# codelion/adaptive-classifier

Measured on NVIDIA H100. Metric: queries/sec predict() bert-base 128-tok, 1M x 768 prototypes, higher is better.
Workload: dtype f16

## Files before the change

### adaptive_classifier_b200/csrc/common.cuh

```cuda
#pragma once

#include <cuda_runtime.h>
#include <cuda.h>
#include <stdint.h>
#include <stdio.h>
#include <string.h>
#include <string>

#include "../../include/adaptive_b200.h"

namespace ac {

void set_error(const char *fmt, ...);
int check_cuda(cudaError_t e, const char *what);

#define AC_CUDA(call)                                                \
    do {                                                             \
        int _rc = ::ac::check_cuda((call), #call);                   \
        if (_rc != 0) return _rc;                                    \
    } while (0)

#define AC_REQUIRE(cond, ...)                                        \
    do {                                                             \
        if (!(cond)) {                                               \
// ... 131 lines not shown
}
__device__ __forceinline__ void wgmma_m64n128_tf32(float (&d)[64], uint64_t a_desc, uint64_t b_desc, uint32_t accumulate) {
    asm volatile(
        "{\n\t"
        ".reg .pred p;\n\t"
        "setp.ne.b32 p, %66, 0;\n\t"
        "wgmma.mma_async.sync.aligned.m64n128k8.f32.tf32.tf32 "
        "{%0, %1, %2, %3, %4, %5, %6, %7, %8, %9, %10, %11, %12, %13, %14, %15, "
        "%16, %17, %18, %19, %20, %21, %22, %23, %24, %25, %26, %27, %28, %29, %30, %31, "
        "%32, %33, %34, %35, %36, %37, %38, %39, %40, %41, %42, %43, %44, %45, %46, %47, "
        "%48, %49, %50, %51, %52, %53, %54, %55, %56, %57, %58, %59, %60, %61, %62, %63}, "
        "%64, %65, p, 1, 1;\n\t"
        "}"
        : "+f"(d[0]), "+f"(d[1]), "+f"(d[2]), "+f"(d[3]), "+f"(d[4]), "+f"(d[5]), "+f"(d[6]), "+f"(d[7]),
          "+f"(d[8]), "+f"(d[9]), "+f"(d[10]), "+f"(d[11]), "+f"(d[12]), "+f"(d[13]), "+f"(d[14]), "+f"(d[15]),
          "+f"(d[16]), "+f"(d[17]), "+f"(d[18]), "+f"(d[19]), "+f"(d[20]), "+f"(d[21]), "+f"(d[22]), "+f"(d[23]),
          "+f"(d[24]), "+f"(d[25]), "+f"(d[26]), "+f"(d[27]), "+f"(d[28]), "+f"(d[29]), "+f"(d[30]), "+f"(d[31]),
          "+f"(d[32]), "+f"(d[33]), "+f"(d[34]), "+f"(d[35]), "+f"(d[36]), "+f"(d[37]), "+f"(d[38]), "+f"(d[39]),
          "+f"(d[40]), "+f"(d[41]), "+f"(d[42]), "+f"(d[43]), "+f"(d[44]), "+f"(d[45]), "+f"(d[46]), "+f"(d[47]),
          "+f"(d[48]), "+f"(d[49]), "+f"(d[50]), "+f"(d[51]), "+f"(d[52]), "+f"(d[53]), "+f"(d[54]), "+f"(d[55]),
          "+f"(d[56]), "+f"(d[57]), "+f"(d[58]), "+f"(d[59]), "+f"(d[60]), "+f"(d[61]), "+f"(d[62]), "+f"(d[63])
        : "l"(a_desc), "l"(b_desc), "r"(accumulate));
}
__device__ __forceinline__ void wgmma_m64n64_f16(float (&d)[32], uint64_t a_desc, uint64_t b_desc, uint32_t accumulate) {
    asm volatile(
        "{\n\t"
        ".reg .pred p;\n\t"
        "setp.ne.b32 p, %34, 0;\n\t"
        "wgmma.mma_async.sync.aligned.m64n64k16.f32.f16.f16 "
        "{%0, %1, %2, %3, %4, %5, %6, %7, %8, %9, %10, %11, %12, %13, %14, %15, "
        "%16, %17, %18, %19, %20, %21, %22, %23, %24, %25, %26, %27, %28, %29, %30, %31}, "
        "%32, %33, p, 1, 1, 0, 0;\n\t"
        "}"
        : "+f"(d[0]), "+f"(d[1]), "+f"(d[2]), "+f"(d[3]), "+f"(d[4]), "+f"(d[5]), "+f"(d[6]), "+f"(d[7]),
          "+f"(d[8]), "+f"(d[9]), "+f"(d[10]), "+f"(d[11]), "+f"(d[12]), "+f"(d[13]), "+f"(d[14]), "+f"(d[15]),
          "+f"(d[16]), "+f"(d[17]), "+f"(d[18]), "+f"(d[19]), "+f"(d[20]), "+f"(d[21]), "+f"(d[22]), "+f"(d[23]),
          "+f"(d[24]), "+f"(d[25]), "+f"(d[26]), "+f"(d[27]), "+f"(d[28]), "+f"(d[29]), "+f"(d[30]), "+f"(d[31])
        : "l"(a_desc), "l"(b_desc), "r"(accumulate));
}
__device__ __forceinline__ void wgmma_m64n32_f16(float (&d)[16], uint64_t a_desc, uint64_t b_desc, uint32_t accumulate) {
    asm volatile(
        "{\n\t"
        ".reg .pred p;\n\t"
        "setp.ne.b32 p, %18, 0;\n\t"
        "wgmma.mma_async.sync.aligned.m64n32k16.f32.f16.f16 "
        "{%0, %1, %2, %3, %4, %5, %6, %7, %8, %9, %10, %11, %12, %13, %14, %15}, "
        "%16, %17, p, 1, 1, 0, 0;\n\t"
        "}"
        : "+f"(d[0]), "+f"(d[1]), "+f"(d[2]), "+f"(d[3]), "+f"(d[4]), "+f"(d[5]), "+f"(d[6]), "+f"(d[7]),
          "+f"(d[8]), "+f"(d[9]), "+f"(d[10]), "+f"(d[11]), "+f"(d[12]), "+f"(d[13]), "+f"(d[14]), "+f"(d[15])
        : "l"(a_desc), "l"(b_desc), "r"(accumulate));
}

template <int NREG>
__device__ __forceinline__ void wgmma_store_acc(const float (&d)[NREG], float *tile, int ld) {
    const int t = threadIdx.x & 127;
    const int r0 = 16 * (t >> 5) + ((t & 31) >> 2), c0 = 2 * (t & 3);
#pragma unroll
    for (int j = 0; j < NREG / 4; ++j) {
        *reinterpret_cast<float2 *>(tile + r0 * ld + 8 * j + c0) = make_float2(d[4 * j], d[4 * j + 1]);
        *reinterpret_cast<float2 *>(tile + (r0 + 8) * ld + 8 * j + c0) = make_float2(d[4 * j + 2], d[4 * j + 3]);
    }
}
__device__ __forceinline__ void acc_row_ld32(const float *p, float (&v)[32]) {
#pragma unroll
    for (int j = 0; j < 32; j += 4) {
        const float4 x = *reinterpret_cast<const float4 *>(p + j);
        v[j] = x.x; v[j + 1] = x.y; v[j + 2] = x.z; v[j + 3] = x.w;
    }
}

int make_tmap_2d(CUtensorMap *out, const void *gptr, int elem_bytes, uint64_t rows, uint64_t cols,
                 uint64_t row_stride_bytes, uint32_t box_rows, uint32_t box_cols);

}
```

### adaptive_classifier_b200/csrc/encoder.cu

```cuda
#include "gemm_tc.cuh"
#include <cuda_fp16.h>
#include <math_constants.h>
#include <algorithm>
#include <array>
#include <type_traits>
#include <vector>

namespace ac {

__device__ __forceinline__ float ex2_approx(float x) {
    float y;
    asm("ex2.approx.ftz.f32 %0, %1;" : "=f"(y) : "f"(x));
    return y;
}
__device__ __forceinline__ float rcp_approx(float x) {
    float y;
    asm("rcp.approx.ftz.f32 %0, %1;" : "=f"(y) : "f"(x));
    return y;
}
__device__ __forceinline__ float gelu_erf(float y) {
    const float ay = fabsf(y);
    const float t = rcp_approx(fmaf(0.3275911f * 0.70710678118654752440f, ay, 1.f));
    float p = fmaf(0.5f * 1.061405429f, t, 0.5f * -1.453152027f);
    p = fmaf(p, t, 0.5f * 1.421413741f);
// ... 475 lines not shown
        if (i < nv) {
            const int col = (lane + 32 * i) * 4;
            const float4 a = __ldg(reinterpret_cast<const float4 *>(word + static_cast<int64_t>(id) * H + col));
            if (!pos) {
                x[i] = a;
                continue;
            }
            const float4 t = __ldg(reinterpret_cast<const float4 *>(type + static_cast<int64_t>(tt) * H + col));
            const float4 q = __ldg(reinterpret_cast<const float4 *>(pos + static_cast<int64_t>(p) * H + col));
            x[i].x = (a.x + t.x) + q.x;
            x[i].y = (a.y + t.y) + q.y;
            x[i].z = (a.z + t.z) + q.z;
            x[i].w = (a.w + t.w) + q.w;
        }
    ln_row(x, nv, H, w, b, eps, lane, F32_OUT ? out_full + static_cast<int64_t>(row) * H : nullptr,
           out_half + static_cast<int64_t>(row) * H);
}

__global__ void cls_normalize_kernel(const float *__restrict__ x, int B, int S, int H, float *__restrict__ out) {
    const int bq = blockIdx.x * (blockDim.x >> 5) + (threadIdx.x >> 5);
    const int lane = threadIdx.x & 31;
    if (bq >= B) return;
    const float *src = x + static_cast<int64_t>(bq) * S * H;
    float s = 0.f;
    for (int i = lane; i < H; i += 32) s = fmaf(src[i], src[i], s);
    const float nrm = fmaxf(sqrtf(warp_sum(s)), 1e-12f);
    for (int i = lane; i < H; i += 32) out[static_cast<int64_t>(bq) * H + i] = src[i] / nrm;
}

__global__ void gather_cls_kernel(const __half *__restrict__ ctx, const float *__restrict__ x, int B, int S, int H,
                                  __half *__restrict__ ctx_cls, float *__restrict__ x_cls) {
    const int bq = blockIdx.x * (blockDim.x >> 5) + (threadIdx.x >> 5);
    const int lane = threadIdx.x & 31;
    if (bq >= B) return;
    const int64_t src = static_cast<int64_t>(bq) * S * H, dst = static_cast<int64_t>(bq) * H;
    for (int i = lane; i < H / 8; i += 32)
        reinterpret_cast<uint4 *>(ctx_cls + dst)[i] = reinterpret_cast<const uint4 *>(ctx + src)[i];
    for (int i = lane; i < H / 4; i += 32)
        reinterpret_cast<float4 *>(x_cls + dst)[i] = reinterpret_cast<const float4 *>(x + src)[i];
}

__global__ void round_copy_kernel(const float *__restrict__ in, float *__restrict__ out, int64_t n, int do_round) {
    const int64_t stride = static_cast<int64_t>(gridDim.x) * blockDim.x;
    for (int64_t i = static_cast<int64_t>(blockIdx.x) * blockDim.x + threadIdx.x; i < n; i += stride)
        out[i] = do_round ? round_tf32(in[i]) : in[i];
}
__global__ void to_half_kernel(const float *__restrict__ in, __half *__restrict__ out, int64_t n) {
    const int64_t stride = static_cast<int64_t>(gridDim.x) * blockDim.x;
    for (int64_t i = static_cast<int64_t>(blockIdx.x) * blockDim.x + threadIdx.x; i < n; i += stride)
        out[i] = __float2half_rn(in[i]);
}

constexpr int ATT_THREADS = 128;
constexpr int ATT_S_LD = 128 + 4;
constexpr int ATT_S_BYTES = 128 * ATT_S_LD * 4;
constexpr int ATT_REGION_BYTES = (ATT_S_BYTES + 1023) / 1024 * 1024;
constexpr int ATT_OFF_VT = ATT_REGION_BYTES, ATT_OFF_BAR = ATT_OFF_VT + 16 * 1024, ATT_OFF_TERM = ATT_OFF_BAR + 64;
template <class Score>
constexpr int ATT_SMEM = ATT_OFF_TERM + Score::SMEM_BLOCK + 1024 ;

template <int DH>
__device__ __forceinline__ void att_scores(const uint8_t *sQ, const uint8_t *sK, float *sS) {
    const uint64_t bd = wgmma_desc_sw128(smem_u32(sK));
#pragma unroll 1
    for (int half = 0; half < 2; ++half) {
        float s[64];
        const uint64_t a = wgmma_desc_sw128(smem_u32(sQ + half * 8192));
        wgmma_fence();
#pragma unroll
        for (int k = 0; k < DH / 16; ++k) wgmma_m64n128_f16(s, a + 2 * k, bd + 2 * k, k != 0);
        wgmma_commit();
        wgmma_wait<0>();
        wgmma_store_acc(s, sS + half * 64 * ATT_S_LD, ATT_S_LD);
    }
}
template <int DH>
__device__ __forceinline__ void att_pv(const uint8_t *sP, const uint8_t *sVt, float (&o)[2][DH / 2], bool accumulate) {
#pragma unroll
    for (int half = 0; half < 2; ++half) {
        wgmma_fence();
#pragma unroll
        for (int slab = 0; slab < 2; ++slab) {
            const uint64_t a = wgmma_desc_sw128(smem_u32(sP + slab * 16384 + half * 8192));
            const uint64_t bd = wgmma_desc_sw128(smem_u32(sVt + slab * 8192));
#pragma unroll
            for (int k = 0; k < 4; ++k) {
                if constexpr (DH == 64) wgmma_m64n64_f16(o[half], a + 2 * k, bd + 2 * k, accumulate || (slab | k) != 0);
                else wgmma_m64n32_f16(o[half], a + 2 * k, bd + 2 * k, accumulate || (slab | k) != 0);
            }
        }
    }
    wgmma_commit();
    wgmma_wait<0>();
}
__device__ __forceinline__ void att_store_p(uint32_t sp_base, int qrow, int c, const uint32_t *pk) {
    const uint32_t prow = sp_base + (c >> 6) * 16384 + (qrow >> 3) * 1024 + (qrow & 7) * 128;
    const int ch0 = (c & 63) >> 3;
#pragma unroll
    for (int ch = 0; ch < 4; ++ch) {
        asm volatile("st.shared.v4.b32 [%0], {%1, %2, %3, %4};" ::"r"(prow + (((ch0 + ch) ^ (qrow & 7)) << 4)),
                     "r"(pk[4 * ch]), "r"(pk[4 * ch + 1]), "r"(pk[4 * ch + 2]), "r"(pk[4 * ch + 3])
                     : "memory");
    }
}
template <int DH>
__device__ __forceinline__ void att_write_row(const float *orow, float inv, __half *dst) {
#pragma unroll
    for (int c = 0; c < DH; c += 8) {
        const float4 a = *reinterpret_cast<const float4 *>(orow + c);
        const float4 b = *reinterpret_cast<const float4 *>(orow + c + 4);
// ... 3 lines not shown
        pk.x = *reinterpret_cast<uint32_t *>(&h0); pk.y = *reinterpret_cast<uint32_t *>(&h1);
        pk.z = *reinterpret_cast<uint32_t *>(&h2); pk.w = *reinterpret_cast<uint32_t *>(&h3);
        *reinterpret_cast<uint4 *>(dst + c) = pk;
    }
}

__device__ __forceinline__ uint32_t band_bits(int q, int k0, int w) {
    if (w <= 0) return 0xffffffffu;
    const int lo = q - w - k0, hi = q + w - k0;
    if (hi < 0 || lo > 31) return 0u;
    const uint32_t up = hi >= 31 ? 0xffffffffu : (2u << hi) - 1u;
    const uint32_t dn = lo <= 0 ? 0xffffffffu : ~((1u << lo) - 1u);
    return up & dn;
}

__device__ __forceinline__ void att_key_bits(const int32_t *mask, int64_t row0, int S, int key0, int q, int window, int lane,
                                             uint32_t (&kmask)[4]) {
#pragma unroll
    for (int w4 = 0; w4 < 4; ++w4) {
        const int key = key0 + 32 * w4 + lane;
        const bool ok = (key < S) && (!mask || mask[row0 + key] != 0);
        kmask[w4] = __ballot_sync(0xffffffffu, ok) & band_bits(q, key0 + 32 * w4, window);
    }
}
__device__ __forceinline__ void att_exp_pack(const float (&r)[32], uint32_t km, float scale_log2, float mxs, float &sum,
                                             uint32_t *pk) {
#pragma unroll
    for (int j = 0; j < 32; j += 2) {
        const float e0 = ((km >> j) & 1u) ? ex2_approx(fmaf(r[j], scale_log2, -mxs)) : 0.f;
        const float e1 = ((km >> (j + 1)) & 1u) ? ex2_approx(fmaf(r[j + 1], scale_log2, -mxs)) : 0.f;
        sum += e0 + e1;
        __half2 hh = __floats2half2_rn(e0, e1);
        pk[j >> 1] = *reinterpret_cast<uint32_t *>(&hh);
    }
}

struct AttCta {
    uint8_t *smem;
    uint8_t *term;
    int tid, h, heads;
    int q0, nblk;
};

struct ScorePlain {
    static constexpr int MIN_DH = 32;
    static constexpr bool ONE_BLOCK = true;
    static constexpr int SCALE_TERMS = 1;
    static constexpr bool EX2_ROWS = false;
    static constexpr int SMEM_BLOCK = 0, SMEM_STREAM = 0;
    __device__ __forceinline__ void init_barriers(const AttCta &) const {}
    __device__ __forceinline__ void begin(const AttCta &) const {}
    __device__ __forceinline__ void add_block_terms(const AttCta &, int) const {}
    __device__ __forceinline__ void row(float (&)[32], const AttCta &, int, float) const {}
    __device__ __forceinline__ void after_pv(const AttCta &, int) const {}
};

struct ScoreRelBias : ScorePlain {
    const float *rel_bias;
    static constexpr int MIN_DH = 64;
    static constexpr bool EX2_ROWS = true;
    static constexpr int ATT_BIAS_OFS = AC_ENCODER_MAX_S - 128;
    static constexpr int SMEM_BLOCK = 1024, SMEM_STREAM = (AC_ENCODER_MAX_S + 128) * 4;
    __device__ __forceinline__ void begin(const AttCta &cta) const {
        const float *row = rel_bias + cta.h * (2 * AC_ENCODER_MAX_S - 1);
        float *sB = reinterpret_cast<float *>(cta.term);
        for (int t = cta.tid; t < 128 * cta.nblk + 127; t += ATT_THREADS)
            sB[t] = __ldg(row + ATT_BIAS_OFS - cta.q0 + t) * 1.44269504088896340736f;
    }
    __device__ __forceinline__ void row(float (&r)[32], const AttCta &cta, int key, float scale_log2) const {
        const float *bq = reinterpret_cast<const float *>(cta.term) + 127 - cta.tid;
#pragma unroll
        for (int j = 0; j < 32; ++j) r[j] = fmaf(r[j], scale_log2, bq[key + j]);
    }
};

template <int DH, class Score>
__global__ void __launch_bounds__(ATT_THREADS)
attention_kernel(const __grid_constant__ CUtensorMap tmap_qk, const __grid_constant__ CUtensorMap tmap_vt,
                 const int32_t *__restrict__ mask, int B, int S, int heads, int H, int window, __half *__restrict__ ctx,
                 const __grid_constant__ Score score) {
    static_assert(Score::ONE_BLOCK && DH >= Score::MIN_DH, "score term not written for this kernel or head dimension");
    static_assert(2 * (ATT_SMEM<Score> + 1024) <= 228 * 1024, "two attention CTAs must fit one SM");
    extern __shared__ uint8_t smem_raw[];
    uint8_t *smem = reinterpret_cast<uint8_t *>((reinterpret_cast<uintptr_t>(smem_raw) + 1023) & ~uintptr_t(1023));
    uint8_t *sQ = smem;
    uint8_t *sK = smem + 16 * 1024;
    float *sS = reinterpret_cast<float *>(smem);
    uint8_t *sP = smem;
    uint8_t *sVt = smem + ATT_OFF_VT;
    uint64_t *bar_load = reinterpret_cast<uint64_t *>(smem + ATT_OFF_BAR);

    const int tid = threadIdx.x, warp = tid >> 5, lane = tid & 31;
    const int b = blockIdx.x / heads, h = blockIdx.x % heads;
    const int64_t row0 = static_cast<int64_t>(b) * S;
    const AttCta cta = {smem, smem + ATT_OFF_TERM, tid, h, heads, 0, 1};

    if (tid == 0) {
        tma_prefetch_desc(&tmap_qk);
        tma_prefetch_desc(&tmap_vt);
        mbar_init(bar_load, 1);
        fence_mbar_init();
    }
    __syncthreads();
    if (tid == 0) {
        mbar_arrive_expect_tx(bar_load, 48 * 1024);
        const int r = static_cast<int>(row0);
        tma_load_2d(sQ, &tmap_qk, bar_load, h * DH, r);
        tma_load_2d(sK, &tmap_qk, bar_load, H + h * DH, r);
        const int vrow = (b * heads + h) * DH;
        tma_load_2d(sVt, &tmap_vt, bar_load, 0, vrow);
        tma_load_2d(sVt + 8 * 1024, &tmap_vt, bar_load, 64, vrow);
    }
    score.begin(cta);
    mbar_wait_guarded(bar_load, 0);
    {
        float s0[64], s1[64];
        const uint64_t bd = wgmma_desc_sw128(smem_u32(sK));
        const uint64_t a0 = wgmma_desc_sw128(smem_u32(sQ)), a1 = wgmma_desc_sw128(smem_u32(sQ + 8192));
        wgmma_fence();
#pragma unroll
        for (int k = 0; k < DH / 16; ++k) wgmma_m64n128_f16(s0, a0 + 2 * k, bd + 2 * k, k != 0);
#pragma unroll
        for (int k = 0; k < DH / 16; ++k) wgmma_m64n128_f16(s1, a1 + 2 * k, bd + 2 * k, k != 0);
        wgmma_commit();
        wgmma_wait<0>();
        __syncthreads();
        wgmma_store_acc(s0, sS, ATT_S_LD);
        wgmma_store_acc(s1, sS + 64 * ATT_S_LD, ATT_S_LD);
    }
    __syncthreads();

    const int qrow = warp * 32 + lane;
    const float *srow = sS + qrow * ATT_S_LD;
    uint32_t kmask[4];
    att_key_bits(mask, row0, S, 0, qrow, window, lane, kmask);
    const float scale_log2 = rsqrtf(static_cast<float>(Score::SCALE_TERMS * DH)) * 1.44269504088896340736f;
    const float sl2 = Score::EX2_ROWS ? 1.f : scale_log2;
    float mx = -CUDART_INF_F;
#pragma unroll 1
    for (int c = 0; c < 128; c += 32) {
        float r[32];
        acc_row_ld32(srow + c, r);
        score.row(r, cta, c, scale_log2);
        const uint32_t km = c == 0 ? kmask[0] : c == 32 ? kmask[1] : c == 64 ? kmask[2] : kmask[3];
#pragma unroll
        for (int j = 0; j < 32; ++j)
            if ((km >> j) & 1u) mx = fmaxf(mx, r[j]);
    }
    float sum = 0.f;
    uint32_t pk[64];
#pragma unroll
    for (int ci = 0; ci < 4; ++ci) {
        float r[32];
        acc_row_ld32(srow + 32 * ci, r);
        score.row(r, cta, 32 * ci, scale_log2);
        att_exp_pack(r, kmask[ci], sl2, mx * sl2, sum, pk + 16 * ci);
    }
    __syncthreads();
    const uint32_t sp_base = smem_u32(sP);
#pragma unroll
    for (int ci = 0; ci < 4; ++ci) att_store_p(sp_base, qrow, 32 * ci, pk + 16 * ci);
    fence_proxy_async_smem();
    __syncthreads();

    float o[2][DH / 2];
    att_pv<DH>(sP, sVt, o, false);
    __syncthreads();
    wgmma_store_acc(o[0], sS, ATT_S_LD);
    wgmma_store_acc(o[1], sS + 64 * ATT_S_LD, ATT_S_LD);
    __syncthreads();
    const float inv = (sum > 0.f) ? 1.f / sum : 0.f;
    if (qrow < S) att_write_row<DH>(srow, inv, ctx + (row0 + qrow) * H + h * DH);
}

constexpr int ATTS_STAGE_BYTES = 16 * 1024;
constexpr int ATTS_OFF_K = 16 * 1024, ATTS_OFF_VT = 48 * 1024, ATTS_OFF_P = 80 * 1024, ATTS_OFF_S = 112 * 1024;
constexpr int ATTS_OFF_BAR = ATTS_OFF_S + ATT_S_BYTES + 128 * 4, ATTS_OFF_TERM = ATTS_OFF_BAR + 2 * 8;
template <class Score>
constexpr int ATTS_SMEM = ATTS_OFF_TERM + Score::SMEM_STREAM + 1024 ;

constexpr int ATTS_POS_DELTAS = 2 * (AC_ENCODER_MAX_S / 128) - 1;

template <bool P2C>
__device__ __forceinline__ void att_rel_term(const uint8_t *sA, const uint8_t *sG, float *sS) {
    const int t = threadIdx.x & 127;
    const int r0 = 16 * (t >> 5) + ((t & 31) >> 2), c0 = 2 * (t & 3);
#pragma unroll 1
    for (int half = 0; half < 2; ++half) {
#pragma unroll 1
        for (int nc = 0; nc < 2; ++nc) {
            float c[64];
            const uint64_t a = wgmma_desc_sw128(smem_u32(sA + half * 8192));
            const uint64_t bd = wgmma_desc_sw128(smem_u32(sG + nc * 16384));
            wgmma_fence();
#pragma unroll
            for (int k = 0; k < 4; ++k) wgmma_m64n128_f16(c, a + 2 * k, bd + 2 * k, k != 0);
            wgmma_commit();
            wgmma_wait<0>();
#pragma unroll
            for (int j = 0; j < 64; ++j) {
                const int row = 64 * half + r0 + 8 * ((j >> 1) & 1);
                const int other = row - (128 * nc + 8 * (j >> 2) + c0 + (j & 1)) + 127;
                if (other >= 0 && other < 128) {
                    float *dst = P2C ? sS + other * ATT_S_LD + row : sS + row * ATT_S_LD + other;
                    *dst += c[j];
                }
            }
        }
    }
}

struct ScoreDisent : ScorePlain {
    CUtensorMap tmap_pos;
    int pos_row0;
    static constexpr int MIN_DH = 64;
    static constexpr bool ONE_BLOCK = false;
    static constexpr int SCALE_TERMS = 3;
    static constexpr int OFF_G = (ATTS_OFF_TERM + 2 * 8 + 1023) / 1024 * 1024 - ATTS_OFF_TERM;
    static constexpr int SMEM_STREAM = OFF_G + 2 * ATTS_STAGE_BYTES;
    __device__ __forceinline__ void issue_pos(const AttCta &cta, int i, int term) const {
        const int row =
            pos_row0 + (((static_cast<int>(blockIdx.y) - i + ATTS_POS_DELTAS / 2) * cta.heads + cta.h) * 2 + term) * 256;
        uint64_t *bar = reinterpret_cast<uint64_t *>(cta.term) + term;
        uint8_t *dst = term ? cta.smem + ATTS_OFF_P : cta.term + OFF_G;
        mbar_arrive_expect_tx(bar, 2 * ATTS_STAGE_BYTES);
// ... 174 lines not shown
}

__global__ void pos_gather_kernel(const float *__restrict__ pos_key, const float *__restrict__ pos_query,
                                  const int32_t *__restrict__ rel_index, int span, int heads, int H, __half *__restrict__ out) {
    const int64_t row = static_cast<int64_t>(blockIdx.x) * 4 + (threadIdx.x >> 6);
    const int col = threadIdx.x & 63;
    const int t = static_cast<int>(row % 256), term = static_cast<int>((row / 256) % 2);
    const int h = static_cast<int>((row / 512) % heads);
    const int64_t ld = row / (512 * static_cast<int64_t>(heads));
    const int d = static_cast<int>(ld % ATTS_POS_DELTAS);
    const int64_t l = ld / ATTS_POS_DELTAS;
    float v = 0.f;
    if (t < 255) {
        const int delta = 128 * (d - ATTS_POS_DELTAS / 2);
        const int r = term ? delta + 127 - t : delta + t - 127;
        const int c = min(max(rel_index[AC_ENCODER_MAX_S - 1 + r], 0), 2 * span - 1);
        v = (term ? pos_query : pos_key)[(l * 2 * span + c) * H + 64 * h + col];
    }
    out[row * 64 + col] = __float2half_rn(v);
}

}

using namespace ac;

struct Layer {
    __half *wqkv = nullptr, *wo = nullptr, *w1 = nullptr, *w2 = nullptr;
    CUtensorMap m_wqkv, m_wo, m_w1, m_w2;
    float *c1qkv = nullptr, *c0qkv = nullptr, *c1f = nullptr, *c0f = nullptr;
    float *bo = nullptr, *b2 = nullptr;
    float *ln_ffn_w = nullptr, *ln_ffn_b = nullptr;
    float *ln_out_w = nullptr, *ln_out_b = nullptr;
    int window = 0;
};

struct ac_encoder {
    ac_encoder_config cfg;
    float *word = nullptr, *pos = nullptr, *type = nullptr, *emb_ln_w = nullptr, *emb_ln_b = nullptr;
    __half *emb_proj_w = nullptr;
    float *emb_proj_b = nullptr;
    CUtensorMap m_emb, m_emb_proj;
    std::vector<Layer> layers;
    __half *w1_last = nullptr;
    float *b1_last = nullptr;
    float *x = nullptr, *tmp = nullptr;
    __half *xh = nullptr, *qk = nullptr, *vT = nullptr, *ctx = nullptr, *ffn = nullptr;
    size_t T = 0;
    size_t vt_elems = 0;
    size_t Bc = 0;
    float *x_cls = nullptr, *tmp_cls = nullptr;
    __half *xh_cls = nullptr, *ctx_cls = nullptr, *ffn_cls = nullptr;
    CUtensorMap m_xh_cls, m_ctx_cls, m_ffn_cls;
    CUtensorMap m_xh, m_ctx, m_ffn, m_qk_att, m_vt_att;
    int vt_B = -1, vt_S = -1;
    CUtensorMap p_w1_last;
    float2 *stats_a = nullptr, *stats_b = nullptr, *stats_id = nullptr, *parts = nullptr;
    float *ones = nullptr, *zeros = nullptr;
    float *rope[2] = {nullptr, nullptr};
    float *rel_bias = nullptr;
    __half *pos_g = nullptr;
    CUtensorMap m_pos;
    std::vector<void *> allocs;
    int last_B = 0, last_S = 0;
    bool last_cls_only = false;
};

static int launch_cls_normalize(const float *x, int B, int S, int H, float *out, cudaStream_t s) {
    const int wpb = 8;
    cls_normalize_kernel<<<(B + wpb - 1) / wpb, wpb * 32, 0, s>>>(x, B, S, H, out);
    AC_LAUNCH_CHECK();
    return AC_OK;
}

struct AttVariant { const void *kernel; int smem; };
enum { ATT_PLAIN64, ATT_PLAIN32, ATT_RELBIAS, ATTS_PLAIN64, ATTS_PLAIN32, ATTS_RELBIAS, ATTS_DISENT, ATT_VARIANTS };
static const AttVariant att_variants[ATT_VARIANTS] = {
    {reinterpret_cast<const void *>(attention_kernel<64, ScorePlain>), ATT_SMEM<ScorePlain>},
    {reinterpret_cast<const void *>(attention_kernel<32, ScorePlain>), ATT_SMEM<ScorePlain>},
    {reinterpret_cast<const void *>(attention_kernel<64, ScoreRelBias>), ATT_SMEM<ScoreRelBias>},
    {reinterpret_cast<const void *>(attention_stream_kernel<64, ScorePlain>), ATTS_SMEM<ScorePlain>},
    {reinterpret_cast<const void *>(attention_stream_kernel<32, ScorePlain>), ATTS_SMEM<ScorePlain>},
    {reinterpret_cast<const void *>(attention_stream_kernel<64, ScoreRelBias>), ATTS_SMEM<ScoreRelBias>},
    {reinterpret_cast<const void *>(attention_stream_kernel<64, ScoreDisent>), ATTS_SMEM<ScoreDisent>},
};

static int launch_attention(ac_encoder *e, const int32_t *mask, int B, int S, int window, bool cls_rows, int layer,
                            cudaStream_t s) {
    const ac_encoder_config &c = e->cfg;
    int H = c.hidden, heads = c.heads;
    const int dh = H / heads;
    AC_REQUIRE(S <= AC_ENCODER_MAX_S || dh == 64, "attention: S=%d > %d needs head_dim 64 (ModernBERT)", S, AC_ENCODER_MAX_S);
    static bool att_attr[64] = {};
    int dev = 0;
    AC_CUDA(cudaGetDevice(&dev));
    if (dev < 0 || dev >= 64 || !att_attr[dev]) {
        for (const AttVariant &v : att_variants)
            AC_CUDA(cudaFuncSetAttribute(v.kernel, cudaFuncAttributeMaxDynamicSharedMemorySize, v.smem));
        if (dev >= 0 && dev < 64) att_attr[dev] = true;
    }
    const int q_blocks = cls_rows ? 1 : (S + 127) / 128;
    const int nq = std::min(S, 128 * q_blocks);
    double keys = 0.0;
    if (window > 0) {
        for (int q = 0; q < nq; ++q) keys += std::min(S - 1, q + window) - std::max(0, q - window) + 1;
    } else {
        keys = static_cast<double>(nq) * S;
    }
    const int slot = prof_begin(PROF_ATTENTION, 4.0 * B * c.heads * keys * dh, 0.0, s);
    const bool streamed = e->pos_g || S > 128;
    ScorePlain plain;
    ScoreRelBias bias;
    ScoreDisent disent;
    void *score = &plain;
    int id = dh == 32 ? (streamed ? ATTS_PLAIN32 : ATT_PLAIN32) : (streamed ? ATTS_PLAIN64 : ATT_PLAIN64);
    if (e->pos_g) {
        disent.tmap_pos = e->m_pos;
        disent.pos_row0 = layer * ATTS_POS_DELTAS * heads * 2 * 256;
        score = &disent;
        id = ATTS_DISENT;
    } else if (e->rel_bias) {
        bias.rel_bias = e->rel_bias;
        score = &bias;
        id = streamed ? ATTS_RELBIAS : ATT_RELBIAS;
    }
    const AttVariant &v = att_variants[id];
    void *args[] = {&e->m_qk_att, &e->m_vt_att, &mask, &B, &S, &heads, &H, &window, &e->ctx, score};
    cudaLaunchKernel(v.kernel, dim3(B * heads, streamed ? q_blocks : 1), dim3(ATT_THREADS), args, v.smem, s);
    prof_end(slot, s);
    AC_LAUNCH_CHECK();
    return AC_OK;
}

template <class T>
static int dev_alloc(ac_encoder *e, T **p, size_t elems) {
    void *q = nullptr;
    AC_CUDA(cudaMalloc(&q, elems * sizeof(T)));
    e->allocs.push_back(q);
    *p = static_cast<T *>(q);
    return AC_OK;
}

static int pack_f32(ac_encoder *e, float **dst, const float *src, size_t n) {
    int rc = dev_alloc(e, dst, n);
    if (rc) return rc;
    round_copy_kernel<<<256, 256>>>(src, *dst, static_cast<int64_t>(n), 0);
    AC_LAUNCH_CHECK();
    return AC_OK;
}
static int pack_f16(ac_encoder *e, __half **dst, const float *src, size_t n) {
    int rc = dev_alloc(e, dst, n);
    if (rc) return rc;
    to_half_kernel<<<256, 256>>>(src, *dst, static_cast<int64_t>(n));
    AC_LAUNCH_CHECK();
    return AC_OK;
}

extern "C" int ac_encoder_destroy(ac_encoder *enc) {
    if (!enc) return AC_OK;
    for (void *p : enc->allocs) cudaFree(p);
    delete enc;
    return AC_OK;
}

static int pack_consumer(ac_encoder *e, int n, const float *const *W, const float *const *bias, const float *gamma,
                         const float *beta, int N, int K, int glu, __half **wp, float **c1, float **c0) {
    const size_t NK = static_cast<size_t>(N) * K;
    int rc;
    if ((rc = dev_alloc(e, wp, n * NK)) || (rc = dev_alloc(e, c1, static_cast<size_t>(n) * N)) ||
        (rc = dev_alloc(e, c0, static_cast<size_t>(n) * N)))
        return rc;
    for (int j = 0; j < n; ++j) {
        pack_defer_kernel<<<(N + 7) / 8, 256>>>(W[j], bias ? bias[j] : nullptr, gamma, beta, N, K, *wp + j * NK, *c1 + j * N,
                                                *c0 + j * N, glu);
        if ((rc = check_cuda(cudaGetLastError(), "pack_defer_kernel"))) return rc;
    }
    return AC_OK;
}

extern "C" int ac_encoder_create(const ac_encoder_config *cfg, const ac_encoder_weights *w, ac_encoder **out) {
// ... 128 lines not shown
            TRY(copy_of(&Layer::bo, w->ao_b, l, H));
            TRY(copy_of(&Layer::ln_ffn_w, w->ao_ln_w, l, H));
            TRY(copy_of(&Layer::ln_ffn_b, w->ao_ln_b, l, H));
            if (const int j = earlier(l, ffn1_src); j >= 0) {
                ly.w1 = e->layers[j].w1, ly.c1f = e->layers[j].c1f, ly.c0f = e->layers[j].c0f;
            } else {
                TRY(pack_consumer(e, 1, &w->ff1_w[l], &w->ff1_b[l], w->ao_ln_w[l], w->ao_ln_b[l], I, H, 0, &ly.w1, &ly.c1f,
                                  &ly.c0f));
            }
            TRY(copy_of(&Layer::w2, w->ff2_w, l, HI));
            TRY(copy_of(&Layer::b2, w->ff2_b, l, H));
            TRY(copy_of(&Layer::ln_out_w, w->out_ln_w, l, H));
            TRY(copy_of(&Layer::ln_out_b, w->out_ln_b, l, H));
        }
        if (cfg->cls_only) {
            TRY(pack_f16(e, &e->w1_last, w->ff1_w[L - 1], HI));
            TRY(pack_f32(e, &e->b1_last, w->ff1_b[L - 1], I));
        }
    }
    TRY(dev_alloc(e, &e->stats_a, T));
    TRY(dev_alloc(e, &e->stats_b, T));
    TRY(dev_alloc(e, &e->stats_id, T));
    TRY(dev_alloc(e, &e->parts, static_cast<size_t>(H / GEMM_EPI_COLS) * T));
    fill_stats_identity_kernel<<<static_cast<unsigned>((T + 255) / 256), 256>>>(e->stats_id, static_cast<int64_t>(T));
    fill_value_kernel<<<(H + 255) / 256, 256>>>(e->ones, H, 1.f);
    fill_value_kernel<<<(nzeros + 255) / 256, 256>>>(e->zeros, nzeros, 0.f);
    TRY(check_cuda(cudaGetLastError(), "deferred-LayerNorm constants"));
    e->vt_elems = 2 * T * H;
    TRY(dev_alloc(e, &e->x, T * H));
    TRY(dev_alloc(e, &e->tmp, T * H));
    TRY(dev_alloc(e, &e->xh, T * H));
    TRY(dev_alloc(e, &e->qk, T * 2 * H));
    TRY(dev_alloc(e, &e->vT, e->vt_elems));
    TRY(dev_alloc(e, &e->ctx, T * H));
    TRY(dev_alloc(e, &e->ffn, T * I));
    e->Bc = T < 16384 ? T : 16384;
    TRY(dev_alloc(e, &e->x_cls, e->Bc * H));
    TRY(dev_alloc(e, &e->tmp_cls, e->Bc * H));
    TRY(dev_alloc(e, &e->xh_cls, e->Bc * H));
    TRY(dev_alloc(e, &e->ctx_cls, e->Bc * H));
    TRY(dev_alloc(e, &e->ffn_cls, e->Bc * I));
    TRY(check_cuda(cudaMemset(e->xh_cls, 0, e->Bc * H * sizeof(__half)), "memset xh_cls"));
    TRY(check_cuda(cudaMemset(e->ctx_cls, 0, e->Bc * H * sizeof(__half)), "memset ctx_cls"));
    TRY(check_cuda(cudaMemset(e->ffn_cls, 0, e->Bc * I * sizeof(__half)), "memset ffn_cls"));
    TRY(check_cuda(cudaMemset(e->qk, 0, T * 2 * H * sizeof(__half)), "memset qk"));
    TRY(check_cuda(cudaMemset(e->vT, 0, e->vt_elems * sizeof(__half)), "memset vT"));
    TRY(check_cuda(cudaMemset(e->xh, 0, T * H * sizeof(__half)), "memset xh"));
    TRY(check_cuda(cudaMemset(e->ctx, 0, T * H * sizeof(__half)), "memset ctx"));
    TRY(check_cuda(cudaMemset(e->ffn, 0, T * I * sizeof(__half)), "memset ffn"));
    TRY(make_tmap_2d(&e->m_xh, e->xh, 2, T, H, static_cast<uint64_t>(H) * 2, GEMM_BLOCK_M, 64));
    TRY(make_tmap_2d(&e->m_ctx, e->ctx, 2, T, H, static_cast<uint64_t>(H) * 2, GEMM_BLOCK_M, 64));
    TRY(make_tmap_2d(&e->m_ffn, e->ffn, 2, T, I, static_cast<uint64_t>(I) * 2, GEMM_BLOCK_M, 64));
    TRY(make_tmap_2d(&e->m_qk_att, e->qk, 2, T, 2 * H, static_cast<uint64_t>(2 * H) * 2, 128, 64));
    TRY(make_tmap_2d(&e->m_xh_cls, e->xh_cls, 2, e->Bc, H, static_cast<uint64_t>(H) * 2, GEMM_BLOCK_M, 64));
    TRY(make_tmap_2d(&e->m_ctx_cls, e->ctx_cls, 2, e->Bc, H, static_cast<uint64_t>(H) * 2, GEMM_BLOCK_M, 64));
    TRY(make_tmap_2d(&e->m_ffn_cls, e->ffn_cls, 2, e->Bc, I, static_cast<uint64_t>(I) * 2, GEMM_BLOCK_M, 64));
    if (e->emb_proj_w) {
        TRY(make_tmap_2d(&e->m_emb, e->ctx, 2, T, E, static_cast<uint64_t>(E) * 2, GEMM_BLOCK_M, 64));
        TRY(make_tmap_2d(&e->m_emb_proj, e->emb_proj_w, 2, H, E, static_cast<uint64_t>(E) * 2, GEMM_BLOCK_N, 64));
    }
    const int n1 = mb ? 2 * I : I;
    for (Layer &ly : e->layers) {
        TRY(make_tmap_2d(&ly.m_wqkv, ly.wqkv, 2, 3 * H, H, static_cast<uint64_t>(H) * 2, GEMM_BLOCK_N, 64));
        TRY(make_tmap_2d(&ly.m_wo, ly.wo, 2, H, H, static_cast<uint64_t>(H) * 2, GEMM_BLOCK_N, 64));
        TRY(make_tmap_2d(&ly.m_w1, ly.w1, 2, n1, H, static_cast<uint64_t>(H) * 2, GEMM_BLOCK_N, 64));
        TRY(make_tmap_2d(&ly.m_w2, ly.w2, 2, H, I, static_cast<uint64_t>(I) * 2, GEMM_BLOCK_N, 64));
    }
    if (cfg->cls_only) TRY(make_tmap_2d(&e->p_w1_last, e->w1_last, 2, n1, H, static_cast<uint64_t>(H) * 2, GEMM_BLOCK_N, 64));
    TRY(check_cuda(cudaDeviceSynchronize(), "encoder_create sync"));
#undef TRY
    *out = e;
    return AC_OK;
}

template <class Epi>
static int launch_linear(const CUtensorMap &ta, const CUtensorMap &tb, int M, int N, int K, const Epi &epi, cudaStream_t s) {
    return launch_gemm_tc<Epi, false, GEMM_KIND_F16>(ta, tb, M, N, K, epi, s);
}

template <bool PRE_LN, Act FFN_ACT>
static int forward_layers(ac_encoder *e, const int32_t *ids, const int32_t *mask, const int32_t *type_ids, int B, int S,
                          float *out_unit_cls, cudaStream_t s) {
    static_assert(PRE_LN == (FFN_ACT == Act::GeGLU), "GeGLU is the pre-LN block's FFN");
    using EpiFfn1 = EpiF16<FFN_ACT, true>;
    using EpiFfn1Rows = EpiF16<FFN_ACT, false>;
    const ac_encoder_config &c = e->cfg;
    const int H = c.hidden, I = c.intermediate, M = B * S;
    const int N1 = PRE_LN ? 2 * I : I;
    const int S_pad = (S + 7) / 8 * 8;
    const int wpb = 8;
    const int row_blocks = (M + wpb - 1) / wpb;
    const int nparts = H / GEMM_EPI_COLS;
    const int64_t pstride = static_cast<int64_t>(e->T);
    const bool cls_tail = c.cls_only && static_cast<size_t>(B) <= e->Bc;
    int rc;
    if (!e->emb_proj_w) {
        embed_ln_kernel<true><<<row_blocks, wpb * 32, 0, s>>>(ids, PRE_LN ? nullptr : type_ids, e->word, e->pos, e->type,
                                                              e->emb_ln_w, e->emb_ln_b, c.ln_eps, B, S, H, c.arch, c.pad_idx,
                                                              c.vocab, c.max_pos, c.type_vocab, e->x, e->xh);
        AC_LAUNCH_CHECK();
    } else {
        const int E = c.embedding_size;
        embed_ln_kernel<false><<<row_blocks, wpb * 32, 0, s>>>(ids, type_ids, e->word, e->pos, e->type, e->emb_ln_w,
                                                               e->emb_ln_b, c.ln_eps, B, S, E, c.arch, c.pad_idx, c.vocab,
                                                               c.max_pos, c.type_vocab, nullptr, e->ctx);
        AC_LAUNCH_CHECK();
// ... 168 lines not shown
```

Measured before the change: 18070.

## Keep attention scores in registers and feed P to wgmma from registers

Rewrites the single-block attention kernel so the QK^T accumulator fragments are masked, softmaxed and packed to half in registers. P then goes straight into register-A wgmma for PV, so the fp32 score tile no longer round-trips through shared memory. The shared-memory footprint shrinks so three CTAs can fit per SM. A CLS-only mode loads and processes just the first 64 query rows via a new 64-row tensor map. This costs more register pressure under the 3-CTA launch bound and more shuffle work for the row reductions.

```diff
diff --git a/adaptive_classifier_b200/csrc/common.cuh b/adaptive_classifier_b200/csrc/common.cuh
--- a/adaptive_classifier_b200/csrc/common.cuh
+++ b/adaptive_classifier_b200/csrc/common.cuh
@@ -207,6 +207,36 @@
         : "l"(a_desc), "l"(b_desc), "r"(accumulate));
 }
 
+__device__ __forceinline__ void wgmma_m64n64_f16_ra(float (&d)[32], const uint32_t *a, uint64_t b_desc, uint32_t accumulate) {
+    asm volatile(
+        "{\n\t"
+        ".reg .pred p;\n\t"
+        "setp.ne.b32 p, %37, 0;\n\t"
+        "wgmma.mma_async.sync.aligned.m64n64k16.f32.f16.f16 "
+        "{%0, %1, %2, %3, %4, %5, %6, %7, %8, %9, %10, %11, %12, %13, %14, %15, "
+        "%16, %17, %18, %19, %20, %21, %22, %23, %24, %25, %26, %27, %28, %29, %30, %31}, "
+        "{%32, %33, %34, %35}, %36, p, 1, 1, 0;\n\t"
+        "}"
+        : "+f"(d[0]), "+f"(d[1]), "+f"(d[2]), "+f"(d[3]), "+f"(d[4]), "+f"(d[5]), "+f"(d[6]), "+f"(d[7]),
+          "+f"(d[8]), "+f"(d[9]), "+f"(d[10]), "+f"(d[11]), "+f"(d[12]), "+f"(d[13]), "+f"(d[14]), "+f"(d[15]),
+          "+f"(d[16]), "+f"(d[17]), "+f"(d[18]), "+f"(d[19]), "+f"(d[20]), "+f"(d[21]), "+f"(d[22]), "+f"(d[23]),
+          "+f"(d[24]), "+f"(d[25]), "+f"(d[26]), "+f"(d[27]), "+f"(d[28]), "+f"(d[29]), "+f"(d[30]), "+f"(d[31])
+        : "r"(a[0]), "r"(a[1]), "r"(a[2]), "r"(a[3]), "l"(b_desc), "r"(accumulate));
+}
+__device__ __forceinline__ void wgmma_m64n32_f16_ra(float (&d)[16], const uint32_t *a, uint64_t b_desc, uint32_t accumulate) {
+    asm volatile(
+        "{\n\t"
+        ".reg .pred p;\n\t"
+        "setp.ne.b32 p, %21, 0;\n\t"
+        "wgmma.mma_async.sync.aligned.m64n32k16.f32.f16.f16 "
+        "{%0, %1, %2, %3, %4, %5, %6, %7, %8, %9, %10, %11, %12, %13, %14, %15}, "
+        "{%16, %17, %18, %19}, %20, p, 1, 1, 0;\n\t"
+        "}"
+        : "+f"(d[0]), "+f"(d[1]), "+f"(d[2]), "+f"(d[3]), "+f"(d[4]), "+f"(d[5]), "+f"(d[6]), "+f"(d[7]),
+          "+f"(d[8]), "+f"(d[9]), "+f"(d[10]), "+f"(d[11]), "+f"(d[12]), "+f"(d[13]), "+f"(d[14]), "+f"(d[15])
+        : "r"(a[0]), "r"(a[1]), "r"(a[2]), "r"(a[3]), "l"(b_desc), "r"(accumulate));
+}
+
 template <int NREG>
 __device__ __forceinline__ void wgmma_store_acc(const float (&d)[NREG], float *tile, int ld) {
     const int t = threadIdx.x & 127;
diff --git a/adaptive_classifier_b200/csrc/encoder.cu b/adaptive_classifier_b200/csrc/encoder.cu
--- a/adaptive_classifier_b200/csrc/encoder.cu
+++ b/adaptive_classifier_b200/csrc/encoder.cu
@@ -551,10 +551,10 @@
 }
 
 constexpr int ATT_THREADS = 128;
+constexpr int ATT_MIN_CTAS = 3;
 constexpr int ATT_S_LD = 128 + 4;
 constexpr int ATT_S_BYTES = 128 * ATT_S_LD * 4;
-constexpr int ATT_REGION_BYTES = (ATT_S_BYTES + 1023) / 1024 * 1024;
-constexpr int ATT_OFF_VT = ATT_REGION_BYTES, ATT_OFF_BAR = ATT_OFF_VT + 16 * 1024, ATT_OFF_TERM = ATT_OFF_BAR + 64;
+constexpr int ATT_OFF_K = 16 * 1024, ATT_OFF_VT = 32 * 1024, ATT_OFF_BAR = 48 * 1024, ATT_OFF_TERM = ATT_OFF_BAR + 64;
 template <class Score>
 constexpr int ATT_SMEM = ATT_OFF_TERM + Score::SMEM_BLOCK + 1024 ;
 
@@ -664,6 +664,7 @@
     __device__ __forceinline__ void begin(const AttCta &) const {}
     __device__ __forceinline__ void add_block_terms(const AttCta &, int) const {}
     __device__ __forceinline__ void row(float (&)[32], const AttCta &, int, float) const {}
+    __device__ __forceinline__ void frag(float (&)[64], const AttCta &, int, float) const {}
     __device__ __forceinline__ void after_pv(const AttCta &, int) const {}
 };
 
@@ -684,27 +685,36 @@
 #pragma unroll
         for (int j = 0; j < 32; ++j) r[j] = fmaf(r[j], scale_log2, bq[key + j]);
     }
+    __device__ __forceinline__ void frag(float (&s)[64], const AttCta &cta, int qa, float scale_log2) const {
+        const float *ba = reinterpret_cast<const float *>(cta.term) + 127 - qa + 2 * (cta.tid & 3), *bb = ba - 8;
+#pragma unroll
+        for (int j = 0; j < 16; ++j) {
+            s[4 * j] = fmaf(s[4 * j], scale_log2, ba[8 * j]);
+            s[4 * j + 1] = fmaf(s[4 * j + 1], scale_log2, ba[8 * j + 1]);
+            s[4 * j + 2] = fmaf(s[4 * j + 2], scale_log2, bb[8 * j]);
+            s[4 * j + 3] = fmaf(s[4 * j + 3], scale_log2, bb[8 * j + 1]);
+        }
+    }
 };
 
 template <int DH, class Score>
-__global__ void __launch_bounds__(ATT_THREADS)
+__global__ void __launch_bounds__(ATT_THREADS, ATT_MIN_CTAS)
 attention_kernel(const __grid_constant__ CUtensorMap tmap_qk, const __grid_constant__ CUtensorMap tmap_vt,
                  const int32_t *__restrict__ mask, int B, int S, int heads, int H, int window, __half *__restrict__ ctx,
-                 const __grid_constant__ Score score) {
+                 const __grid_constant__ Score score, int cls_rows) {
     static_assert(Score::ONE_BLOCK && DH >= Score::MIN_DH, "score term not written for this kernel or head dimension");
-    static_assert(2 * (ATT_SMEM<Score> + 1024) <= 228 * 1024, "two attention CTAs must fit one SM");
+    static_assert(ATT_MIN_CTAS * (ATT_SMEM<Score> + 1024) <= 228 * 1024, "three attention CTAs must fit one SM");
     extern __shared__ uint8_t smem_raw[];
     uint8_t *smem = reinterpret_cast<uint8_t *>((reinterpret_cast<uintptr_t>(smem_raw) + 1023) & ~uintptr_t(1023));
     uint8_t *sQ = smem;
-    uint8_t *sK = smem + 16 * 1024;
-    float *sS = reinterpret_cast<float *>(smem);
-    uint8_t *sP = smem;
+    uint8_t *sK = smem + ATT_OFF_K;
     uint8_t *sVt = smem + ATT_OFF_VT;
     uint64_t *bar_load = reinterpret_cast<uint64_t *>(smem + ATT_OFF_BAR);
 
     const int tid = threadIdx.x, warp = tid >> 5, lane = tid & 31;
     const int b = blockIdx.x / heads, h = blockIdx.x % heads;
     const int64_t row0 = static_cast<int64_t>(b) * S;
+    const int halves = cls_rows ? 1 : 2;
     const AttCta cta = {smem, smem + ATT_OFF_TERM, tid, h, heads, 0, 1};
 
     if (tid == 0) {
@@ -715,74 +725,112 @@
     }
     __syncthreads();
     if (tid == 0) {
-        mbar_arrive_expect_tx(bar_load, 48 * 1024);
+        mbar_arrive_expect_tx(bar_load, (32 + 8 * halves) * 1024);
         const int r = static_cast<int>(row0);
-        tma_load_2d(sQ, &tmap_qk, bar_load, h * DH, r);
+        for (int i = 0; i < halves; ++i) tma_load_2d(sQ + i * 8192, &tmap_qk, bar_load, h * DH, r + 64 * i);
         tma_load_2d(sK, &tmap_qk, bar_load, H + h * DH, r);
+        tma_load_2d(sK + 8192, &tmap_qk, bar_load, H + h * DH, r + 64);
         const int vrow = (b * heads + h) * DH;
         tma_load_2d(sVt, &tmap_vt, bar_load, 0, vrow);
         tma_load_2d(sVt + 8 * 1024, &tmap_vt, bar_load, 64, vrow);
     }
     score.begin(cta);
+    if constexpr (Score::SMEM_BLOCK != 0) __syncthreads();
+    uint32_t kw[4];
+    att_key_bits(mask, row0, S, 0, 0, 0, lane, kw);
+    const float scale_log2 = rsqrtf(static_cast<float>(Score::SCALE_TERMS * DH)) * 1.44269504088896340736f;
+    const float sl2 = Score::EX2_ROWS ? 1.f : scale_log2;
+    const int c0 = 2 * (lane & 3);
+    const uint64_t bk = wgmma_desc_sw128(smem_u32(sK));
     mbar_wait_guarded(bar_load, 0);
-    {
-        float s0[64], s1[64];
-        const uint64_t bd = wgmma_desc_sw128(smem_u32(sK));
-        const uint64_t a0 = wgmma_desc_sw128(smem_u32(sQ)), a1 = wgmma_desc_sw128(smem_u32(sQ + 8192));
+
+#pragma unroll 1
+    for (int half = 0; half < halves; ++half) {
+        float s[64];
+        const uint64_t a = wgmma_desc_sw128(smem_u32(sQ + half * 8192));
         wgmma_fence();
 #pragma unroll
-        for (int k = 0; k < DH / 16; ++k) wgmma_m64n128_f16(s0, a0 + 2 * k, bd + 2 * k, k != 0);
-#pragma unroll
-        for (int k = 0; k < DH / 16; ++k) wgmma_m64n128_f16(s1, a1 + 2 * k, bd + 2 * k, k != 0);
+        for (int k = 0; k < DH / 16; ++k) wgmma_m64n128_f16(s, a + 2 * k, bk + 2 * k, k != 0);
         wgmma_commit();
         wgmma_wait<0>();
-        __syncthreads();
-        wgmma_store_acc(s0, sS, ATT_S_LD);
-        wgmma_store_acc(s1, sS + 64 * ATT_S_LD, ATT_S_LD);
-    }
-    __syncthreads();
-
-    const int qrow = warp * 32 + lane;
-    const float *srow = sS + qrow * ATT_S_LD;
-    uint32_t kmask[4];
-    att_key_bits(mask, row0, S, 0, qrow, window, lane, kmask);
-    const float scale_log2 = rsqrtf(static_cast<float>(Score::SCALE_TERMS * DH)) * 1.44269504088896340736f;
-    const float sl2 = Score::EX2_ROWS ? 1.f : scale_log2;
-    float mx = -CUDART_INF_F;
-#pragma unroll 1
-    for (int c = 0; c < 128; c += 32) {
-        float r[32];
-        acc_row_ld32(srow + c, r);
-        score.row(r, cta, c, scale_log2);
-        const uint32_t km = c == 0 ? kmask[0] : c == 32 ? kmask[1] : c == 64 ? kmask[2] : kmask[3];
-#pragma unroll
-        for (int j = 0; j < 32; ++j)
-            if ((km >> j) & 1u) mx = fmaxf(mx, r[j]);
-    }
-    float sum = 0.f;
-    uint32_t pk[64];
-#pragma unroll
-    for (int ci = 0; ci < 4; ++ci) {
-        float r[32];
-        acc_row_ld32(srow + 32 * ci, r);
-        score.row(r, cta, 32 * ci, scale_log2);
-        att_exp_pack(r, kmask[ci], sl2, mx * sl2, sum, pk + 16 * ci);
-    }
-    __syncthreads();
-    const uint32_t sp_base = smem_u32(sP);
-#pragma unroll
-    for (int ci = 0; ci < 4; ++ci) att_store_p(sp_base, qrow, 32 * ci, pk + 16 * ci);
-    fence_proxy_async_smem();
-    __syncthreads();
-
-    float o[2][DH / 2];
-    att_pv<DH>(sP, sVt, o, false);
-    __syncthreads();
-    wgmma_store_acc(o[0], sS, ATT_S_LD);
-    wgmma_store_acc(o[1], sS + 64 * ATT_S_LD, ATT_S_LD);
-    __syncthreads();
-    const float inv = (sum > 0.f) ? 1.f / sum : 0.f;
-    if (qrow < S) att_write_row<DH>(srow, inv, ctx + (row0 + qrow) * H + h * DH);
+
+        const int qa = 64 * half + 16 * warp + (lane >> 2);
+        score.frag(s, cta, qa, scale_log2);
+        uint32_t km[2][4];
+#pragma unroll
+        for (int i = 0; i < 4; ++i) {
+            km[0][i] = (kw[i] & band_bits(qa, 32 * i, window)) >> c0;
+            km[1][i] = (kw[i] & band_bits(qa + 8, 32 * i, window)) >> c0;
+        }
+        float mx[2] = {-CUDART_INF_F, -CUDART_INF_F};
+#pragma unroll
+        for (int j = 0; j < 16; ++j)
+#pragma unroll
+            for (int e = 0; e < 4; ++e)
+                if ((km[e >> 1][j >> 2] >> (8 * (j & 3) + (e & 1))) & 1u) mx[e >> 1] = fmaxf(mx[e >> 1], s[4 * j + e]);
+        float sum[2] = {0.f, 0.f};
+        uint32_t p[32];
+#pragma unroll
+        for (int r = 0; r < 2; ++r) {
+            mx[r] = fmaxf(mx[r], __shfl_xor_sync(0xffffffffu, mx[r], 1));
+            mx[r] = fmaxf(mx[r], __shfl_xor_sync(0xffffffffu, mx[r], 2));
+            const float mxs = mx[r] * sl2;
+            float pair[16];
+#pragma unroll
+            for (int j = 0; j < 16; ++j) {
+                const uint32_t w = km[r][j >> 2] >> (8 * (j & 3));
+                const float e0 = (w & 1u) ? ex2_approx(fmaf(s[4 * j + 2 * r], sl2, -mxs)) : 0.f;
+                const float e1 = (w & 2u) ? ex2_approx(fmaf(s[4 * j + 2 * r + 1], sl2, -mxs)) : 0.f;
+                pair[j] = e0 + e1;
+                __half2 hh = __floats2half2_rn(e0, e1);
+                p[2 * j + r] = *reinterpret_cast<uint32_t *>(&hh);
+            }
+#pragma unroll
+            for (int j = 0; j < 16; ++j)
+#pragma unroll
+                for (int l = 0; l < 4; ++l) sum[r] += __shfl_sync(0xffffffffu, pair[j], l, 4);
+        }
+
+        float o[DH / 2];
+        wgmma_fence();
+#pragma unroll
+        for (int k = 0; k < 8; ++k) {
+            const uint64_t bd = wgmma_desc_sw128(smem_u32(sVt + (k >> 2) * 8192)) + 2 * (k & 3);
+            if constexpr (DH == 64) wgmma_m64n64_f16_ra(o, p + 4 * k, bd, k != 0);
+            else wgmma_m64n32_f16_ra(o, p + 4 * k, bd, k != 0);
+        }
+        wgmma_commit();
+        wgmma_wait<0>();
+
+        const float inv[2] = {sum[0] > 0.f ? 1.f / sum[0] : 0.f, sum[1] > 0.f ? 1.f / sum[1] : 0.f};
+        const uint32_t stage = smem_u32(sQ + half * 8192 + warp * 2048);
+        const int ra = lane >> 2;
+#pragma unroll
+        for (int j = 0; j < DH / 8; ++j) {
+#pragma unroll
+            for (int r = 0; r < 2; ++r) {
+                __half2 hh = __floats2half2_rn(o[4 * j + 2 * r] * inv[r], o[4 * j + 2 * r + 1] * inv[r]);
+                asm volatile("st.shared.b32 [%0], %1;" ::"r"(stage + (ra + 8 * r) * 128 + ((j ^ ra) << 4) + 2 * c0),
+                             "r"(*reinterpret_cast<uint32_t *>(&hh))
+                             : "memory");
+            }
+        }
+        __syncwarp();
+        constexpr int CPR = DH / 8;
+#pragma unroll
+        for (int i = 0; i < 16 * CPR / 32; ++i) {
+            const int idx = 32 * i + lane, rr = idx / CPR, c = idx % CPR;
+            const int q = 64 * half + 16 * warp + rr;
+            if (q < S && (!cls_rows || q == 0)) {
+                uint4 v;
+                asm volatile("ld.shared.v4.b32 {%0, %1, %2, %3}, [%4];"
+                             : "=r"(v.x), "=r"(v.y), "=r"(v.z), "=r"(v.w)
+                             : "r"(stage + rr * 128 + ((c ^ (rr & 7)) << 4))
+                             : "memory");
+                *reinterpret_cast<uint4 *>(ctx + (row0 + q) * H + h * DH + 8 * c) = v;
+            }
+        }
+    }
 }
 
 constexpr int ATTS_STAGE_BYTES = 16 * 1024;
@@ -1063,6 +1111,7 @@
     __half *xh_cls = nullptr, *ctx_cls = nullptr, *ffn_cls = nullptr;
     CUtensorMap m_xh_cls, m_ctx_cls, m_ffn_cls;
     CUtensorMap m_xh, m_ctx, m_ffn, m_qk_att, m_vt_att;
+    CUtensorMap m_qk_att64;
     int vt_B = -1, vt_S = -1;
     CUtensorMap p_w1_last;
     float2 *stats_a = nullptr, *stats_b = nullptr, *stats_id = nullptr, *parts = nullptr;
@@ -1109,8 +1158,9 @@
             AC_CUDA(cudaFuncSetAttribute(v.kernel, cudaFuncAttributeMaxDynamicSharedMemorySize, v.smem));
         if (dev >= 0 && dev < 64) att_attr[dev] = true;
     }
+    const bool streamed = e->pos_g || S > 128;
     const int q_blocks = cls_rows ? 1 : (S + 127) / 128;
-    const int nq = std::min(S, 128 * q_blocks);
+    const int nq = std::min(S, cls_rows && !streamed ? 64 : 128 * q_blocks);
     double keys = 0.0;
     if (window > 0) {
         for (int q = 0; q < nq; ++q) keys += std::min(S - 1, q + window) - std::max(0, q - window) + 1;
@@ -1118,7 +1168,6 @@
         keys = static_cast<double>(nq) * S;
     }
     const int slot = prof_begin(PROF_ATTENTION, 4.0 * B * c.heads * keys * dh, 0.0, s);
-    const bool streamed = e->pos_g || S > 128;
     ScorePlain plain;
     ScoreRelBias bias;
     ScoreDisent disent;
@@ -1135,7 +1184,9 @@
         id = streamed ? ATTS_RELBIAS : ATT_RELBIAS;
     }
     const AttVariant &v = att_variants[id];
-    void *args[] = {&e->m_qk_att, &e->m_vt_att, &mask, &B, &S, &heads, &H, &window, &e->ctx, score};
+    int cls = cls_rows ? 1 : 0;
+    void *args[] = {streamed ? &e->m_qk_att : &e->m_qk_att64, &e->m_vt_att, &mask, &B, &S, &heads, &H, &window, &e->ctx,
+                    score, &cls};
     cudaLaunchKernel(v.kernel, dim3(B * heads, streamed ? q_blocks : 1), dim3(ATT_THREADS), args, v.smem, s);
     prof_end(slot, s);
     AC_LAUNCH_CHECK();
@@ -1370,6 +1421,7 @@
     TRY(make_tmap_2d(&e->m_ctx, e->ctx, 2, T, H, static_cast<uint64_t>(H) * 2, GEMM_BLOCK_M, 64));
     TRY(make_tmap_2d(&e->m_ffn, e->ffn, 2, T, I, static_cast<uint64_t>(I) * 2, GEMM_BLOCK_M, 64));
     TRY(make_tmap_2d(&e->m_qk_att, e->qk, 2, T, 2 * H, static_cast<uint64_t>(2 * H) * 2, 128, 64));
+    TRY(make_tmap_2d(&e->m_qk_att64, e->qk, 2, T, 2 * H, static_cast<uint64_t>(2 * H) * 2, 64, 64));
     TRY(make_tmap_2d(&e->m_xh_cls, e->xh_cls, 2, e->Bc, H, static_cast<uint64_t>(H) * 2, GEMM_BLOCK_M, 64));
     TRY(make_tmap_2d(&e->m_ctx_cls, e->ctx_cls, 2, e->Bc, H, static_cast<uint64_t>(H) * 2, GEMM_BLOCK_M, 64));
     TRY(make_tmap_2d(&e->m_ffn_cls, e->ffn_cls, 2, e->Bc, I, static_cast<uint64_t>(I) * 2, GEMM_BLOCK_M, 64));
```

New measurement: 18510 (median of 6 runs). 2.4% higher.
